# anacarsi/ss25_Hierarchical_Multiscale_Image_Classification

Hardware: AMD Instinct MI355X
Metric: 224x224 patches/sec (ResNet18 fwd) (higher is better)
Workload: dtype bf16; 1 GPU; resnet18_fwd_872k_patches_bf16; input=uint8 HWC patches resident in HBM, outputs=features[B,512] + logits[B,2] + labels, weights=seeded random init, parallelism=single GPU

## Files before the change

### ss25_hierarchical_multiscale_image_classification_amd/csrc/block16_c64.h

```cpp
#pragma once
#include "halo16.h"

namespace hipac {

typedef __attribute__((ext_vector_type(2))) short s16x2;
__device__ __forceinline__ unsigned relu_pk(unsigned v) {
  return __builtin_bit_cast(unsigned, __builtin_elementwise_max(__builtin_bit_cast(s16x2, v), s16x2{0, 0}));
}

constexpr int kBlkRing = 30;
constexpr int kBlkXPitch = 18 * 128;
constexpr int kBlkIPitch = 16 * 128;
constexpr int kBlkXBytes = 32 * kBlkXPitch + 512;
constexpr int kBlkIBytes = 32 * kBlkIPitch + 256;
constexpr int kBlkRsBytes = 2 * 6144 + 2 * 4096;

#ifndef HIPAC_BLK16_AHEAD
#define HIPAC_BLK16_AHEAD 1
#endif

template <typename T, int NP, int PITCH>
__device__ __forceinline__ void c64_strip16_mfma(const typename Elem<T>::frag (&wreg)[9][2][2], const int (&lb)[NP][3],
                                                 const float* __restrict__ bl, f32x4 (&acc)[2 * NP][2]) {
  using frag = typename Elem<T>::frag;
  constexpr int NR = 2 * NP;
#pragma unroll
  for (int t = 0; t < 2; ++t) {
    const f32x4 b = *reinterpret_cast<const f32x4*>(bl + 16 * t);
#pragma unroll
    for (int i = 0; i < NR; ++i) acc[i][t] = b;
  }
  asm volatile("s_waitcnt lgkmcnt(0)" ::: "memory");
  constexpr int AH = HIPAC_BLK16_AHEAD;
  frag fr[AH + 1][NR];
  auto rd = [&](auto S, auto I) {
    constexpr int s = decltype(S)::value, i = decltype(I)::value;
    constexpr int tap = s >> 1, kk = s & 1, kh = tap / 3, kw = tap % 3;
    lds_read16<((i & 1) + kh) * PITCH>(fr[s % (AH + 1)][i], (unsigned)(lb[i >> 1][kw] ^ (kk << 6)));
  };
  __builtin_amdgcn_s_setprio(1);
  static_for<AH>([&](auto S) { static_for<NR>([&](auto I) { rd(S, I); }); });
  static_for<18>([&](auto S) {
    constexpr int s = decltype(S)::value, tap = s >> 1, kk = s & 1;
    static_for<NR>([&](auto I) {
      constexpr int i = decltype(I)::value;
      if constexpr (s + AH < 18) rd(std::integral_constant<int, s + AH>{}, I);
      constexpr int full = (18 - 1 - s < AH - 1 ? 18 - 1 - s : AH - 1);
      wait_lgkmcnt<(NR - 1 - i) + full * NR + (s + AH < 18 ? i + 1 : 0)>();
      Asm16<T>::mfma(acc[i][0], wreg[tap][kk][0], fr[s % (AH + 1)][i]);
      Asm16<T>::mfma(acc[i][1], wreg[tap][kk][1], fr[s % (AH + 1)][i]);
    });
  });
  __builtin_amdgcn_s_setprio(0);
  asm volatile("s_nop 7\n\ts_nop 7\n\ts_nop 3" ::: "memory");
}

template <typename T>
__global__ __launch_bounds__(512, 2) void block16_c64_kernel(const T* __restrict__ in, const T* __restrict__ w1,
                                                             const float* __restrict__ b1, const T* __restrict__ w2,
                                                             const float* __restrict__ b2, T* __restrict__ out,
                                                             int n_img) {
  using E = Elem<T>;
  using frag = typename E::frag;
  using vec4 = typename E::vec4;
  constexpr int H = 56, W = 56, C = 64, RING = kBlkRing, XP = kBlkXPitch, IP = kBlkIPitch;
  __shared__ __attribute__((aligned(1024))) unsigned char smem[kBlkXBytes + kBlkIBytes + kBlkRsBytes + 512];
  unsigned char* const Xr = smem;
  unsigned char* const Ir = smem + kBlkXBytes;
  float* const Bl = reinterpret_cast<float*>(smem + kBlkXBytes + kBlkIBytes + kBlkRsBytes);

  const int tid = threadIdx.x, lane = tid & 63;
  const int wave = __builtin_amdgcn_readfirstlane(tid >> 6);
  const int team = wave >> 2, tw = wave & 3, nh = tw & 1, mh = tw >> 1;
  const int n16 = lane & 15, g = lane >> 4;
  const int lx = n16 < 4 ? 2 * n16 : (n16 < 12 ? 2 * n16 - 7 : 2 * n16 - 16);
  unsigned char* const Rw = smem + kBlkXBytes + kBlkIBytes + (mh == 0 ? nh * 6144 : 2 * 6144 + nh * 4096);

  if (tid < 64) Bl[tid] = b1[tid];
  else if (tid < 128) Bl[tid] = b2[tid - 64];

  const int xcd = blockIdx.x & 7, slot = blockIdx.x >> 3, nslots = gridDim.x >> 3;
  const int n_x = n_img > xcd ? (n_img - xcd + 7) >> 3 : 0;
  const int nst = 4 * n_x;
  const int ns = nst > slot ? (nst - slot + nslots - 1) / nslots : 0;
  if (ns == 0) return;

  frag wreg[9][2][2];
  {
    const char* wb = reinterpret_cast<const char*>(team ? w2 : w1) + (size_t)(nh * 32 + n16) * (9 * C * 2) + 16 * g;
#pragma unroll
    for (int tap = 0; tap < 9; ++tap)
#pragma unroll
      for (int kk = 0; kk < 2; ++kk)
#pragma unroll
        for (int t = 0; t < 2; ++t) wreg[tap][kk][t] = *reinterpret_cast<const frag*>(wb + t * 16 * (9 * C * 2) + tap * 128 + kk * 64);
  }

  const rsrc_t x_rsrc = make_rsrc(in, n_img * (H * W * C * 2));

  constexpr int NKP = 5;
  int relo[NKP];
#pragma unroll
  for (int kp = 0; kp < NKP; ++kp) {
    const int q = 8 * (tw + 4 * kp) + (lane >> 3);
    const int rr = (q * 3641) >> 16;
    const int j = q - 18 * rr;
    const int c = (lane & 7) ^ ((j >> 1) & 7);
    relo[kp] = (((rr * W + j) << 7) + (c << 4)) | (j < 2 ? 1 : 0) | (j >= 16 ? 2 : 0) | (rr == 0 ? 4 : 0) | (rr >= 1 ? 8 : 0);
  }
  auto x_rows = [&](int img, int x0, int L0, int rb, int np, int rowmask) {
    const int sb = ((img * H + L0 - 1) * W + x0 - 2) << 7;
    const int smask = (x0 == 0 ? 1 : 0) | (x0 == 42 ? 2 : 0) | rowmask;
    static_for<NKP>([&](auto KP) {
      constexpr int kp = decltype(KP)::value;
      const int p = tw + 4 * kp;
      if (p < np) {
        asm volatile("" : "+v"(relo[kp]));
        const int off = (relo[kp] & smask) ? (int)0x80000000 : (relo[kp] & ~15) + sb;
        buffer_load_lds16(x_rsrc, Xr + rb * XP + p * 1024, off, 0);
      }
    });
  };
  auto x_group = [&](int img, int x0, int gq) {
    const int rb = 8 * gq >= RING ? 8 * gq - RING : 8 * gq;
    x_rows(img, x0, 8 * gq, rb, gq == 7 ? 5 : 18, gq == 0 ? 4 : (gq == 7 ? 8 : 0));
    if (gq == 3) x_rows(img, x0, RING, 0, 5, 0);
  };
  auto strip_img = [&](int k) { return (((slot + k * nslots) >> 2) << 3) + xcd; };
  auto strip_x0 = [&](int k) { return ((slot + k * nslots) & 3) * 14; };

  const int lds_base = (int)(unsigned)(size_t)(__attribute__((address_space(3))) unsigned char*)smem;
  int la[3];
#pragma unroll
  for (int kw = 0; kw < 3; ++kw) {
    const int j = lx + kw;
    la[kw] = (j << 7) + (((((j >> 1) & 7)) ^ g) << 4) + (team ? kBlkXBytes : 0) + lds_base;
  }
  const int iw_lane = (lx << 7) + ((g & 1) << 3);
  const int iw_pos = ((nh << 2) + (g >> 1)) ^ ((lx >> 1) & 7);
  const float* const bl = Bl + team * 64 + nh * 32 + 4 * g;

#pragma unroll
  for (int tap = 0; tap < 9; ++tap)
#pragma unroll
    for (int kk = 0; kk < 2; ++kk)
#pragma unroll
      for (int t = 0; t < 2; ++t) asm volatile("" ::"v"(wreg[tap][kk][t]));
  if (team == 0) {
    x_group(strip_img(0), strip_x0(0), 0);
    x_group(strip_img(0), strip_x0(0), 1);
    wait_vmcnt<0>();
  }
  asm volatile("s_waitcnt lgkmcnt(0)" ::: "memory");
  __builtin_amdgcn_s_barrier();

  const int n_steps = 7 * ns;
  f32x4 acc[4][2];
  int pend_n = 0, pend_y = 0;
  const int rs_px = lane >> 2;
  const int rs_off = (((rs_px < 14 ? rs_px : 13)) * C + nh * 32 + 8 * ((lane & 3) ^ ((rs_px >> 2) & 3))) * 2;
  auto fetch_resid = [&](int pix0, int y0, int sl) {
    const int sb = (pix0 + y0 * W) << 7;
#pragma unroll
    for (int rho = 0; rho < 2; ++rho) buffer_load_lds16(x_rsrc, Rw + sl * 2048 + rho * 1024, rs_off + rho * (W * C * 2), sb);
  };
  const int rs_rd = lx * 64 + 8 * (g & 1);
  const int rs_sw = (lx >> 2) & 3;
  const int out_lane = (lx * C + nh * 32 + 16 * (g & 1) + 8 * (g >> 1)) * 2;
  auto epilogue_b = [&](auto A0, int pix0, int y0, int sl) {
    constexpr int a0 = decltype(A0)::value;
#pragma unroll
    for (int rho = 0; rho < 2; ++rho) {
      unsigned P[2][2];
#pragma unroll
      for (int t = 0; t < 2; ++t) {
        const vec4 rv = *reinterpret_cast<const vec4*>(Rw + sl * 2048 + rho * 1024 + rs_rd + (((2 * t + (g >> 1)) ^ rs_sw) << 4));
        const f32x4& a = acc[a0 + rho][t];
        P[t][0] = relu_pk(PackPair<T>::pack_rn(a[0] + (float)rv[0], a[1] + (float)rv[1]));
        P[t][1] = relu_pk(PackPair<T>::pack_rn(a[2] + (float)rv[2], a[3] + (float)rv[3]));
      }
      permlane16_swap(P[0][0], P[1][0]);
      permlane16_swap(P[0][1], P[1][1]);
      char* const dst = reinterpret_cast<char*>(out) + ((size_t)(unsigned)(pix0 + (y0 + rho) * W) << 7) + out_lane;
      if (lx < 14) store16_out(dst, u32x4{P[0][0], P[0][1], P[1][0], P[1][1]});
    }
  };
  int pend_pix = 0, pend_sl = 0;
  auto flush_b = [&]() {
    if (pend_n) {
      wait_vmcnt<0>();
      epilogue_b(std::integral_constant<int, 0>{}, pend_pix, pend_y, pend_sl);
      if (pend_n == 2) epilogue_b(std::integral_constant<int, 2>{}, pend_pix, pend_y + 2, pend_sl + 1);
      pend_n = 0;
    }
  };
  auto step_barrier = [&]() {
    asm volatile("s_waitcnt lgkmcnt(0)" ::: "memory");
    __builtin_amdgcn_s_barrier();
  };
  if (team == 0) {
    for (int G = 0; G <= n_steps; ++G) {
      if (G < n_steps) {
        const int k = G / 7, m = G - 7 * k;
        const int img = strip_img(k), x0 = strip_x0(k);
        if (m <= 4) x_group(img, x0, m + 2);
        else if (m == 5) {
          x_group(img, x0, 7);
          if (k + 1 < ns) x_group(strip_img(k + 1), strip_x0(k + 1), 0);
        } else if (k + 1 < ns) x_group(strip_img(k + 1), strip_x0(k + 1), 1);
        if (m == 0 || m == 6)
          *reinterpret_cast<u32x2*>(Ir + (m == 0 ? 0 : 27) * IP + tw * 512 + lane * 8) = u32x2{0u, 0u};
        const int y0a = 8 * m + 4 * mh;
        int lb[2][3];
#pragma unroll
        for (int p = 0; p < 2; ++p) {
          const int y0 = y0a + 2 * p;
          const int wbase = (y0 >= RING ? y0 - RING : y0) * XP;
#pragma unroll
          for (int kw = 0; kw < 3; ++kw) lb[p][kw] = la[kw] + wbase;
        }
        c64_strip16_mfma<T, 2, XP>(wreg, lb, bl, acc);
        const bool col_ok = !((x0 == 0 && lx == 0) || (x0 == 42 && lx == 15));
#pragma unroll
        for (int i = 0; i < 4; ++i) {
          const int Lr = y0a + i + 1;
          const bool twice = Lr == RING || Lr == RING + 1;
          unsigned char* const dst = Ir + (Lr >= RING ? Lr - RING : Lr) * IP + iw_lane;
          unsigned char* const dst2 = Ir + Lr * IP + iw_lane;
#pragma unroll
          for (int t = 0; t < 2; ++t) {
            u32x2 pk;
            pk[0] = relu_pk(PackPair<T>::pack_rn(acc[i][t][0], acc[i][t][1]));
            pk[1] = relu_pk(PackPair<T>::pack_rn(acc[i][t][2], acc[i][t][3]));
            if (!col_ok) pk = u32x2{0u, 0u};
            *reinterpret_cast<u32x2*>(dst + ((iw_pos ^ (2 * t)) << 4)) = pk;
            if (twice) *reinterpret_cast<u32x2*>(dst2 + ((iw_pos ^ (2 * t)) << 4)) = pk;
          }
        }
      }
      wait_vmcnt<0>();
      step_barrier();
    }
  } else {
    for (int G = 0; G <= n_steps; ++G) {
      flush_b();
      if (G >= 1) {
        const int k = (G - 1) / 7, mp = G - 7 * k;
        int yp = 8 * mp - 10 + 4 * mh, ys = -1;
        bool has_pair = true;
        if (mp == 1) {
          if (mh == 0) yp = 0;
          else has_pair = false, ys = 4;
        } else if (mp == 7) {
          if (mh == 0) yp = 46, ys = 50;
          else yp = 52;
        }
        const int pix0 = strip_img(k) * (H * W) + strip_x0(k);
        if (has_pair) {
          fetch_resid(pix0, yp, 0);
          fetch_resid(pix0, yp + 2, 1);
        }
        if (ys >= 0) fetch_resid(pix0, ys, has_pair ? 2 : 0);
        pend_pix = pix0;
        if (has_pair) {
          int lb[2][3];
#pragma unroll
          for (int p = 0; p < 2; ++p) {
            const int y0 = yp + 2 * p;
            const int wbase = (y0 >= RING ? y0 - RING : y0) * IP;
#pragma unroll
            for (int kw = 0; kw < 3; ++kw) lb[p][kw] = la[kw] + wbase;
          }
          c64_strip16_mfma<T, 2, IP>(wreg, lb, bl, acc);
          pend_n = 2, pend_y = yp, pend_sl = 0;
        }
        if (ys >= 0) {
          flush_b();
          int lb[1][3];
          const int wbase = (ys >= RING ? ys - RING : ys) * IP;
#pragma unroll
          for (int kw = 0; kw < 3; ++kw) lb[0][kw] = la[kw] + wbase;
          f32x4(&acc1)[2][2] = reinterpret_cast<f32x4(&)[2][2]>(acc[0]);
          c64_strip16_mfma<T, 1, IP>(wreg, lb, bl, acc1);
          pend_n = 1, pend_y = ys, pend_sl = has_pair ? 2 : 0;
        }
      }
      step_barrier();
    }
    flush_b();
  }
}

}
```

Before: 317,200 patches/s.

## Fold residual LDS reads into conv MFMA pipeline and use buffer stores

The residual tile is now read from LDS as an extra 19th read group inside the MFMA read-ahead pipeline, and added to the accumulators right after the conv instead of in the epilogue. This removes the separate wait_vmcnt and LDS reads at flush time. The output store becomes a raw buffer store, with an out-of-range offset masking columns 14-15 in place of a branch. It risks wrong lgkmcnt accounting from the new reads-behind helper and stalls from the wait_vmcnt placed inside the MFMA loop.

```diff
diff --git a/ss25_hierarchical_multiscale_image_classification_amd/csrc/block16_c64.h b/ss25_hierarchical_multiscale_image_classification_amd/csrc/block16_c64.h
--- a/ss25_hierarchical_multiscale_image_classification_amd/csrc/block16_c64.h
+++ b/ss25_hierarchical_multiscale_image_classification_amd/csrc/block16_c64.h
@@ -7,6 +7,14 @@
 __device__ __forceinline__ unsigned relu_pk(unsigned v) {
   return __builtin_bit_cast(unsigned, __builtin_elementwise_max(__builtin_bit_cast(s16x2, v), s16x2{0, 0}));
 }
+
+#if defined(__HIP_DEVICE_COMPILE__)
+__device__ __forceinline__ void buffer_store16(rsrc_t rs, u32x4 v, int voffset, int soffset) {
+  __builtin_amdgcn_raw_buffer_store_b128(v, rs, voffset, soffset, 0);
+}
+#else
+__device__ inline void buffer_store16(rsrc_t, u32x4, int, int) {}
+#endif
 
 constexpr int kBlkRing = 30;
 constexpr int kBlkXPitch = 18 * 128;
@@ -18,10 +26,19 @@
 #ifndef HIPAC_BLK16_AHEAD
 #define HIPAC_BLK16_AHEAD 1
 #endif
-
-template <typename T, int NP, int PITCH>
+template <int OFF>
+__device__ __forceinline__ void lds_read8(u32x2& f, unsigned addr) {
+  asm volatile("ds_read_b64 %0, %1 offset:%2" : "=v"(f) : "v"(addr), "n"(OFF));
+}
+constexpr int blk16_reads_behind(int nr, int ah, int ngr, int s, int i) {
+  int n = nr - 1 - i;
+  for (int q = s + 1; q < s + ah && q < ngr; ++q) n += nr * (q == 18 ? 2 : 1);
+  return n + (s + ah < ngr ? (i + 1) * (s + ah == 18 ? 2 : 1) : 0);
+}
+
+template <typename T, int NP, int PITCH, bool TAIL>
 __device__ __forceinline__ void c64_strip16_mfma(const typename Elem<T>::frag (&wreg)[9][2][2], const int (&lb)[NP][3],
-                                                 const float* __restrict__ bl, f32x4 (&acc)[2 * NP][2]) {
+                                                 const float* __restrict__ bl, f32x4 (&acc)[2 * NP][2], const unsigned (&rs)[2]) {
   using frag = typename Elem<T>::frag;
   constexpr int NR = 2 * NP;
 #pragma unroll
@@ -33,26 +50,47 @@
   asm volatile("s_waitcnt lgkmcnt(0)" ::: "memory");
   constexpr int AH = HIPAC_BLK16_AHEAD;
   frag fr[AH + 1][NR];
+  [[maybe_unused]] u32x2 rv[NR][2];
+  constexpr int NGR = TAIL ? 19 : 18;
   auto rd = [&](auto S, auto I) {
     constexpr int s = decltype(S)::value, i = decltype(I)::value;
-    constexpr int tap = s >> 1, kk = s & 1, kh = tap / 3, kw = tap % 3;
-    lds_read16<((i & 1) + kh) * PITCH>(fr[s % (AH + 1)][i], (unsigned)(lb[i >> 1][kw] ^ (kk << 6)));
-  };
+    if constexpr (s < 18) {
+      constexpr int tap = s >> 1, kk = s & 1, kh = tap / 3, kw = tap % 3;
+      lds_read16<((i & 1) + kh) * PITCH>(fr[s % (AH + 1)][i], (unsigned)(lb[i >> 1][kw] ^ (kk << 6)));
+    } else {
+      if constexpr (i == 0) wait_vmcnt<0>();
+      lds_read8<i * 1024>(rv[i][0], rs[0]);
+      lds_read8<i * 1024>(rv[i][1], rs[1]);
+    }
+  };
+  static_assert(AH >= 1 && AH < 18, "read-ahead depth");
   __builtin_amdgcn_s_setprio(1);
   static_for<AH>([&](auto S) { static_for<NR>([&](auto I) { rd(S, I); }); });
   static_for<18>([&](auto S) {
     constexpr int s = decltype(S)::value, tap = s >> 1, kk = s & 1;
     static_for<NR>([&](auto I) {
       constexpr int i = decltype(I)::value;
-      if constexpr (s + AH < 18) rd(std::integral_constant<int, s + AH>{}, I);
-      constexpr int full = (18 - 1 - s < AH - 1 ? 18 - 1 - s : AH - 1);
-      wait_lgkmcnt<(NR - 1 - i) + full * NR + (s + AH < 18 ? i + 1 : 0)>();
+      if constexpr (s + AH < NGR) rd(std::integral_constant<int, s + AH>{}, I);
+      wait_lgkmcnt<blk16_reads_behind(NR, AH, NGR, s, i)>();
       Asm16<T>::mfma(acc[i][0], wreg[tap][kk][0], fr[s % (AH + 1)][i]);
       Asm16<T>::mfma(acc[i][1], wreg[tap][kk][1], fr[s % (AH + 1)][i]);
     });
   });
   __builtin_amdgcn_s_setprio(0);
   asm volatile("s_nop 7\n\ts_nop 7\n\ts_nop 3" ::: "memory");
+  if constexpr (TAIL) {
+    using vec4 = typename Elem<T>::vec4;
+    wait_lgkmcnt<0>();
+#pragma unroll
+    for (int i = 0; i < NR; ++i)
+#pragma unroll
+      for (int t = 0; t < 2; ++t) {
+        asm_landed(rv[i][t]);
+        const vec4 r = __builtin_bit_cast(vec4, rv[i][t]);
+#pragma unroll
+        for (int e = 0; e < 4; ++e) acc[i][t][e] += (float)r[e];
+      }
+  }
 }
 
 template <typename T>
@@ -62,7 +100,6 @@
                                                              int n_img) {
   using E = Elem<T>;
   using frag = typename E::frag;
-  using vec4 = typename E::vec4;
   constexpr int H = 56, W = 56, C = 64, RING = kBlkRing, XP = kBlkXPitch, IP = kBlkIPitch;
   __shared__ __attribute__((aligned(1024))) unsigned char smem[kBlkXBytes + kBlkIBytes + kBlkRsBytes + 512];
   unsigned char* const Xr = smem;
@@ -164,33 +201,33 @@
 #pragma unroll
     for (int rho = 0; rho < 2; ++rho) buffer_load_lds16(x_rsrc, Rw + sl * 2048 + rho * 1024, rs_off + rho * (W * C * 2), sb);
   };
-  const int rs_rd = lx * 64 + 8 * (g & 1);
-  const int rs_sw = (lx >> 2) & 3;
-  const int out_lane = (lx * C + nh * 32 + 16 * (g & 1) + 8 * (g >> 1)) * 2;
-  auto epilogue_b = [&](auto A0, int pix0, int y0, int sl) {
+  unsigned rs_lane[2];
+#pragma unroll
+  for (int t = 0; t < 2; ++t)
+    rs_lane[t] = (unsigned)(lds_base + (int)(Rw - smem) + lx * 64 + 8 * (g & 1) + (((2 * t + (g >> 1)) ^ ((lx >> 2) & 3)) << 4));
+  const rsrc_t o_rsrc = make_rsrc(out, n_img * (H * W * C * 2));
+  const int out_lane = lx < 14 ? (lx * C + nh * 32 + 16 * (g & 1) + 8 * (g >> 1)) * 2 : (int)0x80000000;
+  auto epilogue_b = [&](auto A0, int pix0, int y0) {
     constexpr int a0 = decltype(A0)::value;
 #pragma unroll
     for (int rho = 0; rho < 2; ++rho) {
       unsigned P[2][2];
 #pragma unroll
       for (int t = 0; t < 2; ++t) {
-        const vec4 rv = *reinterpret_cast<const vec4*>(Rw + sl * 2048 + rho * 1024 + rs_rd + (((2 * t + (g >> 1)) ^ rs_sw) << 4));
         const f32x4& a = acc[a0 + rho][t];
-        P[t][0] = relu_pk(PackPair<T>::pack_rn(a[0] + (float)rv[0], a[1] + (float)rv[1]));
-        P[t][1] = relu_pk(PackPair<T>::pack_rn(a[2] + (float)rv[2], a[3] + (float)rv[3]));
+        P[t][0] = relu_pk(PackPair<T>::pack_rn(a[0], a[1]));
+        P[t][1] = relu_pk(PackPair<T>::pack_rn(a[2], a[3]));
       }
       permlane16_swap(P[0][0], P[1][0]);
       permlane16_swap(P[0][1], P[1][1]);
-      char* const dst = reinterpret_cast<char*>(out) + ((size_t)(unsigned)(pix0 + (y0 + rho) * W) << 7) + out_lane;
-      if (lx < 14) store16_out(dst, u32x4{P[0][0], P[0][1], P[1][0], P[1][1]});
-    }
-  };
-  int pend_pix = 0, pend_sl = 0;
+      buffer_store16(o_rsrc, u32x4{P[0][0], P[0][1], P[1][0], P[1][1]}, out_lane, (pix0 + (y0 + rho) * W) << 7);
+    }
+  };
+  int pend_pix = 0;
   auto flush_b = [&]() {
     if (pend_n) {
-      wait_vmcnt<0>();
-      epilogue_b(std::integral_constant<int, 0>{}, pend_pix, pend_y, pend_sl);
-      if (pend_n == 2) epilogue_b(std::integral_constant<int, 2>{}, pend_pix, pend_y + 2, pend_sl + 1);
+      epilogue_b(std::integral_constant<int, 0>{}, pend_pix, pend_y);
+      if (pend_n == 2) epilogue_b(std::integral_constant<int, 2>{}, pend_pix, pend_y + 2);
       pend_n = 0;
     }
   };
@@ -219,7 +256,7 @@
 #pragma unroll
           for (int kw = 0; kw < 3; ++kw) lb[p][kw] = la[kw] + wbase;
         }
-        c64_strip16_mfma<T, 2, XP>(wreg, lb, bl, acc);
+        c64_strip16_mfma<T, 2, XP, false>(wreg, lb, bl, acc, rs_lane);
         const bool col_ok = !((x0 == 0 && lx == 0) || (x0 == 42 && lx == 15));
 #pragma unroll
         for (int i = 0; i < 4; ++i) {
@@ -256,11 +293,12 @@
           else yp = 52;
         }
         const int pix0 = strip_img(k) * (H * W) + strip_x0(k);
+        const int sl_s = has_pair ? 2 : 0;
         if (has_pair) {
           fetch_resid(pix0, yp, 0);
           fetch_resid(pix0, yp + 2, 1);
         }
-        if (ys >= 0) fetch_resid(pix0, ys, has_pair ? 2 : 0);
+        if (ys >= 0) fetch_resid(pix0, ys, sl_s);
         pend_pix = pix0;
         if (has_pair) {
           int lb[2][3];
@@ -271,8 +309,8 @@
 #pragma unroll
             for (int kw = 0; kw < 3; ++kw) lb[p][kw] = la[kw] + wbase;
           }
-          c64_strip16_mfma<T, 2, IP>(wreg, lb, bl, acc);
-          pend_n = 2, pend_y = yp, pend_sl = 0;
+          c64_strip16_mfma<T, 2, IP, true>(wreg, lb, bl, acc, rs_lane);
+          pend_n = 2, pend_y = yp;
         }
         if (ys >= 0) {
           flush_b();
@@ -281,8 +319,9 @@
 #pragma unroll
           for (int kw = 0; kw < 3; ++kw) lb[0][kw] = la[kw] + wbase;
           f32x4(&acc1)[2][2] = reinterpret_cast<f32x4(&)[2][2]>(acc[0]);
-          c64_strip16_mfma<T, 1, IP>(wreg, lb, bl, acc1);
-          pend_n = 1, pend_y = ys, pend_sl = has_pair ? 2 : 0;
+          const unsigned rs_s[2] = {rs_lane[0] + sl_s * 2048, rs_lane[1] + sl_s * 2048};
+          c64_strip16_mfma<T, 1, IP, true>(wreg, lb, bl, acc1, rs_s);
+          pend_n = 1, pend_y = ys;
         }
       }
       step_barrier();
```

After: 319,700 patches/s (median of 6 runs). Within noise of the previous version (+0.8%).
